# quadjr/aframe-gaussian-splatting

Measured on AMD Instinct MI355X. Metric: frames/sec @1920x1080 (sort+project+bin+blend per frame, 1M-splat train.splat-shaped scene), higher is better.
Workload: dtype f32

## Files before the change

### aframe-gaussian-splatting_amd/capi.py

```python
import ctypes as C
import os
import sys

import numpy as np

from . import build as _build

GS_OK = 0
E_BADARG, E_PLY_HEADER, E_PLY_PROP, E_HIP, E_OOM, E_NODEVICE, E_STATE, E_PLY_DATA, E_RETRY = -1, -2, -3, -4, -5, -6, -7, -8, -9
RENDER_FLIP_Y, RENDER_COUNT_FRAGS, RENDER_NO_EARLY_OUT, RENDER_ASYNC, RENDER_COUNT_EVALUATED = 1, 2, 4, 8, 16
OPT_PROFILE, OPT_TERMINATION, OPT_NEAR_PERMILLE, OPT_RECORD_STAGED, OPT_PIPELINE_DEPTH, OPT_WIDE_PAIRS, OPT_ENQUEUE_THREADS = 1, 2, 3, 4, 5, 6, 7
OPT_COMM_SELF_COPY = 8
OPT_BLEND_SPLIT = 9
OPT_FRAME_BATCH = 10
OPT_SORT_NEAR = 11
OPT_COMM_TRANSPORT = 12
OPT_AUTO_RETRY = 13
OPT_SORT_SHARE = 15
OPT_BINNING = 16
OPT_SUBTILE = 17
OPT_ROW_WALK = 18
OPT_SH_DEGREE = 19
OPT_ANTIALIAS = 20
OPT_SEG_COUNT = 21
OPT_SORT_NEAR_FORCE = 22
SORT_WHOLE, SORT_HISTOGRAM, SORT_SPEC, SORT_TAIL, SORT_STASH = 0, 1, 2, 3, 4
TRANSPORT_RCCL, TRANSPORT_INPROC = 0, 1
COMM_ID_BYTES = 128
BUF_CENTER_SCALE, BUF_COV_COLOR, BUF_SORT_ROWS, BUF_SORTED, BUF_PROJECTED, BUF_TILE_COUNT, BUF_TILE_STATS, BUF_UNSAT_MASK = 0, 1, 2, 3, 4, 5, 6, 7
BUF_SH = 8
BUF_STATE = 9
STATE_HIDDEN, STATE_SELECTED = 1, 2
SELECT_INVERT = 1

EXPORTS = [
    "gs_create", "gs_destroy", "gs_last_error", "gs_version", "gs_device_count", "gs_clear", "gs_push_splat", "gs_push_matrices", "gs_load_ply",
    "gs_ply_to_splat", "gs_ply_to_splat_gpu", "gs_count", "gs_sort", "gs_render", "gs_render_device", "gs_render_stereo", "gs_set_scene", "gs_sync",
    "gs_set_stream", "gs_frame_stream", "gs_frame_status_device", "gs_frame_lane", "gs_lane_stream", "gs_wait_stream", "gs_stream_wait_frame",
    "gs_model_view_matrix", "gs_projection_matrix", "gs_tick_uniforms", "gs_focal", "gs_scaled_size", "gs_set_option",
    "gs_get_stats", "gs_download",
    "gs_comm_unique_id", "gs_comm_init", "gs_comm_destroy", "gs_partition", "gs_render_gathered", "gs_read_gathered",
    "gs_host_alloc", "gs_host_free", "gs_sort_for", "gs_sort_gathered", "gs_gathered_size", "gs_sort_begin", "gs_sort_poll",
    "gs_create_multi", "gs_multi_destroy", "gs_multi_last_error", "gs_multi_devices", "gs_multi_ctx", "gs_multi_clear",
    "gs_multi_push_splat", "gs_multi_load_ply", "gs_multi_count", "gs_multi_set_option", "gs_multi_sort", "gs_multi_render",
    "gs_multi_render_device", "gs_multi_read", "gs_multi_sync",
    "gs_ply_sh", "gs_ply_sh_host", "gs_push_sh", "gs_sh_count", "gs_sh_eval", "gs_sh_eval_unrounded", "gs_camera_in_object", "gs_multi_push_sh",
    "gs_render_surface", "gs_render_surface_device", "gs_pick",
    "gs_antialias_factor",
    "gs_set_state", "gs_set_state_ids", "gs_state_count", "gs_select_box", "gs_select_sphere", "gs_select_rect", "gs_compact",
    "gs_sort_inspect",
    "gs_multi_set_state", "gs_multi_set_state_ids", "gs_multi_select_box", "gs_multi_select_sphere", "gs_multi_select_rect", "gs_multi_compact",
]
SURFACE_NONE = 0xFFFFFFFF

# ... 767 lines not shown
```

### aframe-gaussian-splatting_amd/csrc/gs_api.hip

```cpp
#include <stddef.h>
#include <stdlib.h>
#include <condition_variable>
#include <deque>
#include <functional>
#include <mutex>
#include <new>
#include <thread>
#include <set>
#include <vector>
#include "gs_internal.h"
#include "gs_ply.h"
#include "gs_sh.h"
#include "gs_host_tables.h"

static thread_local char g_create_err[512] = "";
thread_local char *gs_tl_err = nullptr;

#define CHECK_CTX(ctx) do { if (!(ctx)) return GS_E_BADARG; } while (0)
#define FAIL(code, ...) do { snprintf(GS_ERRBUF(ctx), GS_ERRLEN, __VA_ARGS__); return (code); } while (0)

template <typename T> static int dev_alloc(gs_ctx *ctx, T **p, size_t count)
{
    *p = nullptr;
    if (!count) count = 1;
// ... 711 lines not shown
}

GS_API const char *gs_last_error(const gs_ctx *ctx) { return ctx ? ctx->err : g_create_err; }

GS_API int gs_create(int device, gs_ctx **out)
{
    if (!out) return GS_E_BADARG;
    *out = nullptr;
    int ndev = 0;
    hipError_t e = hipGetDeviceCount(&ndev);
    if (e != hipSuccess || ndev <= 0) {
        snprintf(g_create_err, sizeof g_create_err, "no HIP device available (%s); this library has no CPU fallback",
                 e != hipSuccess ? hipGetErrorString(e) : "device count 0");
        return GS_E_NODEVICE;
    }
    if (device < 0 || device >= ndev) {
        snprintf(g_create_err, sizeof g_create_err, "device %d out of range (have %d)", device, ndev);
        return GS_E_BADARG;
    }
    gs_ctx *ctx = new (std::nothrow) gs_ctx();
    if (!ctx) { snprintf(g_create_err, sizeof g_create_err, "out of host memory"); return GS_E_OOM; }
    memset(ctx, 0, sizeof *ctx);
    ctx->device = device; ctx->renderable = true; ctx->t_eps = 1.0f / 1024.0f; gs_share_reset_create(ctx->share);
    ctx->lanes[0] = ctx; ctx->pipe_depth = 3; ctx->enqueue_threads = true; ctx->frame_batch = 1; ctx->exec = ctx; ctx->sort_near_opt = 1; ctx->auto_retry = true; ctx->subtile_opt = 1; ctx->row_walk_opt = 1; ctx->seg_count_opt = 1;
    { const char *e = getenv("GS_SPEC_STASH"); ctx->near_spec_opt = !(e && e[0] == '0'); }
#define CREATE_HIP(call) do { hipError_t _e = (call); if (_e != hipSuccess) {                                              \
        snprintf(g_create_err, sizeof g_create_err, "%s failed: %s", #call, hipGetErrorString(_e)); gs_destroy(ctx);      \
        return GS_E_HIP; } } while (0)
    CREATE_HIP(hipSetDevice(device));
    CREATE_HIP(init_frame_resources(ctx));
    {
        double tab[GS_POW10_ENTRIES];
        gs_build_pow10_table(tab);
        CREATE_HIP(hipMalloc((void **)&ctx->pow10tab, sizeof tab));
        CREATE_HIP(hipMemcpy(ctx->pow10tab, tab, sizeof tab, hipMemcpyHostToDevice));
    }
#undef CREATE_HIP
    *out = ctx;
    return GS_OK;
}

GS_API int gs_destroy(gs_ctx *ctx)
{
    if (!ctx) return GS_OK;
    (void)hipSetDevice(ctx->device);
    (void)gs_comm_destroy(ctx);
    for (int i = GS_MAX_LANES - 1; i >= 1; i--)
// ... 1157 lines not shown
        ctx->cur = 0; ctx->rot = 0; ctx->cur_async = false;
        return prepare_lanes(ctx);
    case GS_OPT_FRAME_BATCH:
        if (value != 1 && value != 2) FAIL(GS_E_BADARG, "frame batch must be 1 (off) or 2");
        GS_HIP(hipSetDevice(ctx->device));
        TRY(drain_all(ctx));
        ctx->frame_batch = (int)value;
        ctx->cur = 0; ctx->rot = 0; ctx->cur_async = false;
        return prepare_lanes(ctx);
    case GS_OPT_SUBTILE:
        if (value < 0 || value > 2) FAIL(GS_E_BADARG, "sub-tile lists: 0 (off), 1 (where splats are small) or 2 (always)");
        ctx->subtile_opt = (int)value;
        return GS_OK;
    case GS_OPT_ROW_WALK:
        if (value < 0 || value > 2) FAIL(GS_E_BADARG, "row walk: 0 (off), 1 (where splats are large) or 2 (always)");
        ctx->row_walk_opt = (int)value;
        return GS_OK;
    case GS_OPT_SEG_COUNT:
        if (value < 0 || value > 2) FAIL(GS_E_BADARG, "segment counts: 0 (never), 1 (where tile rows hold many runs) or 2 (always)");
        GS_HIP(hipSetDevice(ctx->device));
        TRY(drain_all(ctx));
        ctx->seg_count_opt = (int)value;
        return GS_OK;
    case GS_OPT_SH_DEGREE:
        if (value < 0 || value > GS_SH_MAX_DEGREE) FAIL(GS_E_BADARG, "spherical-harmonics degree: 0 (off) to 3");
        ctx->sh_opt = (int)value;
        return GS_OK;
    case GS_OPT_ANTIALIAS:
        if (value != 0 && value != 1) FAIL(GS_E_BADARG, "anti-aliased splats: 0 (off) or 1 (opacity compensated for the 0.3 px^2 dilation)");
        ctx->aa_opt = (int)value;
        return GS_OK;
    case GS_OPT_SORT_NEAR:
        if (value < 0 || value > 2) FAIL(GS_E_BADARG, "near-only sorts: 0 (off), 1 (scenes of 4 M splats and more) or 2 (always)");
        GS_HIP(hipSetDevice(ctx->device));
        TRY(drain_all(ctx));
        ctx->sort_near_opt = (int)value;
        return GS_OK;
    case GS_OPT_SORT_NEAR_FORCE:
        if (value < 0 || value > 0xFFFFFFFFll) FAIL(GS_E_BADARG, "forced near-only sorts: 0 (the policy decides) or the positions every sort without an index list is asked for");
        GS_HIP(hipSetDevice(ctx->device));
        TRY(drain_all(ctx));
        ctx->sort_near_force = (uint32_t)value;
        return GS_OK;
    default: FAIL(GS_E_BADARG, "unknown option %d", option);
    }
}
// ... 71 lines not shown
                                        hipMemcpyDeviceToHost));
        return GS_OK;
    }
    if (which == GS_BUF_STATE) {
        if (nbytes > ctx->edit_n) FAIL(GS_E_BADARG, "buffer %d holds %zu bytes, %zu requested", which, ctx->edit_n, nbytes);
        if (nbytes) GS_HIP(hipMemcpy(out, ctx->edit_state, nbytes, hipMemcpyDeviceToHost));
        return GS_OK;
    }
    if (which == GS_BUF_SH) {
        const size_t K = (size_t)gsm::sh_coefs(ctx->sh_deg), KS = (size_t)gsm::sh_channel_stride(ctx->sh_deg);
        if (nbytes > ctx->sh_n * 3 * K * 4 || nbytes % (K * 4)) FAIL(GS_E_BADARG, "buffer %d holds %zu bytes, %zu requested", which, ctx->sh_n * 3 * K * 4, nbytes);
        if (nbytes) GS_HIP(hipMemcpy2D(out, K * 4, ctx->sh, KS * 4, K * 4, nbytes / (K * 4), hipMemcpyDeviceToHost));
        return GS_OK;
    }
    switch (which) {
    case GS_BUF_SORT_ROWS: src = ctx->sort_rows; have = ctx->n * 16; break;
    case GS_BUF_SORTED:
        if (L->have_sort && L->sort_near_req) { TRY(lane_rc(ctx, L, ensure_full_sort(L))); GS_HIP(hipStreamSynchronize(L->stream)); }
        src = L->sorted; have = L->have_sort ? V * 4 : 0; break;
    case GS_BUF_PROJECTED: src = L->proj; have = L->have_sort ? V * 32 : 0; break;
    case GS_BUF_TILE_COUNT: src = L->tile_count; have = L->have_sort ? V * 4 : 0; break;
    case GS_BUF_TILE_STATS: src = L->tile_range; have = L->tile_cap * 8; break;
    case GS_BUF_UNSAT_MASK: src = L->unsat_mask; have = L->mask_cap * 4; break;
    default: FAIL(GS_E_BADARG, "unknown buffer %d", which);
    }
    if (nbytes > have) FAIL(GS_E_BADARG, "buffer %d holds %zu bytes, %zu requested", which, have, nbytes);
    if (nbytes && (!ctx->renderable && (which == GS_BUF_CENTER_SCALE || which == GS_BUF_COV_COLOR)))
        FAIL(GS_E_STATE, "context holds worker rows only");
    if (nbytes) GS_HIP(hipMemcpy(out, src, nbytes, hipMemcpyDeviceToHost));
    return GS_OK;
}

}
```

### aframe-gaussian-splatting_amd/csrc/gs_internal.h

```cpp
#pragma once
#include <hip/hip_runtime.h>
#include <stdint.h>
#include <stdio.h>
#include <string.h>
#include <type_traits>
#include "../../include/gs_splat.h"
#include "gs_device_math.h"
#include "gs_share.h"

#if defined(__HIP_DEVICE_COMPILE__) && !defined(__gfx950__)
#error "libgs_splat_hip is written for gfx950 (MI355X) only: build with --offload-arch=gfx950"
#endif

#define GS_TILE 16
#define GS_BLOCK 256
#define GS_CHUNK_S 2048
#define GS_CHUNK_L 4096
#ifndef GS_RADIX_LARGE_N
#define GS_RADIX_LARGE_N (3u << 20)
#endif
#define GS_RADIX_MAX_BINS 512
#define GS_TOUCH_PRIVATE_WORDS 16u
#define GS_STATUS_RING 64u
#define GS_NEED_WORDS 32u
// ... 157 lines not shown
    uint32_t *hist;  size_t hist_cap;
    uint32_t *radix_aux; size_t aux_cap;
    uint32_t *spine; size_t spine_cap;
    uint32_t *msd_grp; size_t msd_grp_cap;
    uint32_t *msd_tab;

    gsm::Projected *proj;
    uint2 *rect;
    uint32_t *tile_count;
    uint2 *emit_extra;
    float *zwin;
    float *scene_depth; uint32_t *scene_rgba; int scene_w, scene_h;
    uint2 *pair_a, *pair_b; size_t pair_cap;
    uint32_t blend_split_min;
    uint32_t pair_hint;
    uint32_t run_hint;
    uint32_t *row_cnt; size_t row_cnt_cap;
    uint2 *row_tot; size_t row_tot_cap;
    int *seg_diff;
    int bin_mode;
    int subtile_opt;
    int row_walk_opt;
    int seg_count_opt;
    uint32_t last_pairs, last_visible;
    uint2 *tile_range; size_t tile_cap;
    uint8_t *fb; size_t fb_cap;
    uint8_t *surf_buf; size_t surf_cap;
    struct GsComm *comm;
    uint8_t *gstage; size_t gstage_cap;
    uint8_t *gframe[2]; size_t gframe_cap[2];
    int gviews, gw[2], gh[2];
    float4 *state; size_t state_cap;
    uint32_t *unsat_mask; size_t mask_cap;
    GsShare share;
    GsShareLane share_lane;
    unsigned long long *part_min, *part_max;
    uint32_t *part_cnt, *part_valid, *part_vis;
    GsControl *ctl;
    GsControl *ctl_host;

    bool profile;
    bool profile_blend_only;
    uint32_t profile_every;
    uint32_t profile_tick;
    uint32_t record_staged;
    bool wide_pairs;
// ... 111 lines not shown
```

### aframe-gaussian-splatting_amd/csrc/gs_render.hip

```cpp
#include "gs_internal.h"
#include "gs_sh.h"

namespace {

#define GS_DPP_ADD(V, CTRL, ROWS) (V) += (uint32_t)__builtin_amdgcn_update_dpp(0, (int)(V), (CTRL), (ROWS), 0xF, false)
__device__ __forceinline__ uint32_t row16_sum(uint32_t v)
{
#ifdef GS_DEBUG_DPP_MAX
    const uint32_t v0_ = v;
#endif
    GS_DPP_ADD(v, 0xB1, 0xF);
    GS_DPP_ADD(v, 0x4E, 0xF);
    GS_DPP_ADD(v, 0x141, 0xF);
    GS_DPP_ADD(v, 0x140, 0xF);
#ifdef GS_DEBUG_DPP_MAX
    { uint32_t c = v0_; for (int m = 8; m >= 1; m >>= 1) c += __shfl_xor(c, m, 16); if (c != v) __builtin_trap(); }
#endif
    return v;
}
__device__ __forceinline__ uint32_t wave_sum(uint32_t v)
{
#ifdef GS_DEBUG_DPP_MAX
    uint32_t c_ = v; for (int m = 32; m >= 1; m >>= 1) c_ += __shfl_xor(c_, m, 64);
#endif
// ... 596 lines not shown
    __syncthreads();
    if (tid == 0) {
        const uint32_t total = I > 0xFFFFFFFFull ? 0xFFFFFFFFu : (uint32_t)I;
        ctl->vis_total = 0; ctl->n_emit_extra = 0;
        ctl->n_runs = (ROUND == 0 ? 0u : ctl->n_runs) + runs;
        if (ROUND == 0) { ctl->n_visible = 0; ctl->n_pairs_frame = 0; ctl->want_frame = 0; }
        else { ctl->unsat_round0 = ctl->unsat_count; if (ctl->unsat_count) ctl->unsat_events += 1; }
        ctl->j_lo = j_lo; ctl->j_hi = j_hi;
        ctl->scan_total = total;
        ctl->want_frame = (ctl->want_frame + total < total) ? 0xFFFFFFFFu : ctl->want_frame + total;
        if (ctl->want_frame > ctl->max_total) ctl->max_total = ctl->want_frame;
        if (total > pair_cap) { ctl->pair_overflow = 1; ctl->overflow_sticky = 1; ctl->n_pairs = 0; }
        else if (ROUND == 0) { ctl->pair_overflow = 0; ctl->n_pairs = total; }
        else ctl->n_pairs = ctl->pair_overflow ? 0u : total;
        ctl->n_visible += s_vis; ctl->n_pairs_frame += ctl->n_pairs;
        if (ROUND == 0 && near_count != 0xFFFFFFFFu) ctl->unsat_count = 0;
        if (last_round) {
            ctl->acc_frames += 1; ctl->acc_sorted += ctl->n_kept; ctl->acc_visible += ctl->n_visible; ctl->acc_pairs += ctl->n_pairs_frame;
        }
    }
    __syncthreads();
}

template <int ROUND>
__device__ __forceinline__ void k_emit_runs_body(const gsm::Projected *__restrict__ proj, const uint2 *__restrict__ rect,
                                                 const uint32_t *__restrict__ tile_count, const uint32_t *__restrict__ row_cnt,
                                                 const uint2 *__restrict__ row_tot, const GsFrameUniforms &u,
                                                 uint32_t *__restrict__ run_geom, uint32_t *__restrict__ run_ref,
                                                 const uint32_t *__restrict__ mask, GsControl *ctl, uint32_t pair_cap, uint2 *__restrict__ row_runs,
                                                 const uint32_t *__restrict__ part_vis, uint32_t nparts, int last_round)
{
    __shared__ float s_rec[GS_BLOCK][6];
    __shared__ uint32_t s_rows[GS_BLOCK], s_t[GS_BLOCK];
    __shared__ unsigned long long s_m[GS_BLOCK][4];
    __shared__ uint32_t s_rowrun[GS_BLOCK + 1], s_rowpair[GS_BLOCK + 1], s_base[GS_BLOCK];
    __shared__ uint32_t s_nbig, s_nmid;
    __shared__ unsigned long long s_p[4];
    const uint32_t tid = threadIdx.x;
    const int lane = threadIdx.x & 63, w = threadIdx.x >> 6;
    const uint32_t tiles_y = (uint32_t)u.tiles_y;
    const unsigned long long I = row_prefixes<false>(row_tot, tiles_y, s_rowrun, s_rowpair, nullptr, s_p);
    uint32_t j_lo, j_hi;
    round_range<ROUND>(ctl, u.near_count, j_lo, j_hi);
    const bool overflow = I > pair_cap || (ROUND == 1 && ctl->pair_overflow);
    if (blockIdx.x == 0) {
        round_books<ROUND>(ctl, I, s_rowrun[GS_BLOCK], j_lo, j_hi, u.near_count, part_vis, nparts, last_round, pair_cap);
        if (ROUND == 0 && tid < tiles_y) row_runs[tid] = make_uint2(s_rowrun[tid], overflow ? 0u : s_rowrun[tid + 1] - s_rowrun[tid]);
    }
    if (overflow) return;
    const uint32_t nchunks = (j_hi - j_lo + GS_BLOCK - 1) / GS_BLOCK;
    for (uint32_t c = blockIdx.x; c < nchunks; c += gridDim.x) {
        s_m[tid][0] = 0ull; s_m[tid][1] = 0ull; s_m[tid][2] = 0ull; s_m[tid][3] = 0ull;
        if (tid == 0) { s_nbig = 0; s_nmid = 0; }
        if (tid < tiles_y) s_base[tid] = s_rowrun[tid] + row_cnt[(size_t)tid * u.rc_stride + c];
        __syncthreads();
        const uint32_t j = j_lo + c * GS_BLOCK + tid;
        const uint32_t cnt = j < j_hi ? tile_count[j] : 0u;
        bool own = false;
        uint32_t ty0 = 0, ty1 = 0;
        gsm::Projected p;
        p.cx = p.cy = p.ax = p.ay = p.bx = p.by = 0.0f;
        uint32_t own_runs = 0, own_present = 0;
        if (cnt) {
            const uint2 rc = rect[j];
            if (rc.x & (1u << 14)) {
                own = true;
                ty0 = rc.x >> 16; ty1 = ty0 + ((rc.x >> 15) & 1u);
                own_runs = rc.y; own_present = (rc.x >> 12) & 3u;
            } else {
                const float4 *src = reinterpret_cast<const float4 *>(proj + j);
                const float4 ra = src[0]; const float2 rb = *reinterpret_cast<const float2 *>(src + 1);
                p.cx = ra.x; p.cy = ra.y; p.ax = ra.z; p.ay = ra.w; p.bx = rb.x; p.by = rb.y;
                ty0 = rc.x >> 16; ty1 = rc.y >> 16;
                const uint32_t q = (ty1 - ty0 >= 16) ? (GS_BLOCK - 1u - atomicAdd(&s_nbig, 1u)) : atomicAdd(&s_nmid, 1u);
                s_rec[q][0] = p.cx; s_rec[q][1] = p.cy; s_rec[q][2] = p.ax; s_rec[q][3] = p.ay; s_rec[q][4] = p.bx; s_rec[q][5] = p.by;
                s_rows[q] = ty0 | (ty1 << 16); s_t[q] = tid;
            }
        }
        __syncthreads();
        const uint32_t nmid = s_nmid, nbig = s_nbig;
#define GS_RUN_ONE(PP, EE, T, TY, FN) do { uint32_t a_, n_;                                                                       \
            gsm::splat_tile_row(PP, EE, (int)(TY), u.H, u.x0, u.x1b, a_, n_);                                                     \
            if (n_ && (ROUND == 0 || mask_count(mask + (TY) * u.mask_words, a_, n_))) { FN((T), (TY), a_, n_); } } while (0)
#define GS_RUN_PASS(FN) do {                                                                                                      \
            if (own) {                                                                                                            \
                for (uint32_t ty = ty0; ty <= ty1; ty++) if ((own_present >> (ty - ty0)) & 1u) {                                  \
                    const uint32_t r_ = own_runs >> (16u * (ty - ty0)), a_ = r_ & 0xFFu, n_ = ((r_ >> 8) & 0xFFu) + 1u;           \
                    if (ROUND == 0 || mask_count(mask + ty * u.mask_words, a_, n_)) { FN(tid, ty, a_, n_); } } }                  \
            for (uint32_t mi = (uint32_t)w * 4u + ((uint32_t)lane >> 4); mi < nmid; mi += 16u) {                                  \
                gsm::Projected q;                                                                                                 \
                q.cx = s_rec[mi][0]; q.cy = s_rec[mi][1]; q.ax = s_rec[mi][2]; q.ay = s_rec[mi][3]; q.bx = s_rec[mi][4]; q.by = s_rec[mi][5]; \
                gsm::EllipseRows e; gsm::ellipse_rows_setup(q, e);                                                                \
                const uint32_t ty = (s_rows[mi] & 0xFFFFu) + ((uint32_t)lane & 15u);                                              \
                if (ty <= (s_rows[mi] >> 16)) GS_RUN_ONE(q, e, s_t[mi], ty, FN); }                                                \
            for (uint32_t bq = (uint32_t)w; bq < nbig; bq += 4u) {                                                                \
                const uint32_t bi = GS_BLOCK - 1u - bq;                                                                           \
                gsm::Projected q;                                                                                                 \
                q.cx = s_rec[bi][0]; q.cy = s_rec[bi][1]; q.ax = s_rec[bi][2]; q.ay = s_rec[bi][3]; q.bx = s_rec[bi][4]; q.by = s_rec[bi][5]; \
                gsm::EllipseRows e; gsm::ellipse_rows_setup(q, e);                                                                \
                for (uint32_t ty = (s_rows[bi] & 0xFFFFu) + (uint32_t)lane; ty <= (s_rows[bi] >> 16); ty += 64u) GS_RUN_ONE(q, e, s_t[bi], ty, FN); } \
        } while (0)
#define GS_RUN_MARK(T, TY, A, N) atomicOr(&s_m[TY][(T) >> 6], 1ull << ((T) & 63u))
        GS_RUN_PASS(GS_RUN_MARK);
        __syncthreads();
#define GS_RUN_WRITE(T, TY, A, N) do { const uint32_t wq_ = (T) >> 6;                                                             \
            uint32_t rank_ = (uint32_t)__popcll(s_m[TY][wq_] & ((1ull << ((T) & 63u)) - 1ull));                                   \
            for (uint32_t k_ = 0; k_ < wq_; k_++) rank_ += (uint32_t)__popcll(s_m[TY][k_]);                                       \
            const uint32_t slot_ = s_base[TY] + rank_;                                                                            \
            run_geom[slot_] = (A) | ((N) << 16); run_ref[slot_] = j_lo + c * GS_BLOCK + (T); } while (0)
        GS_RUN_PASS(GS_RUN_WRITE);
#undef GS_RUN_WRITE
#undef GS_RUN_MARK
#undef GS_RUN_PASS
#undef GS_RUN_ONE
        __syncthreads();
    }
}

template <int ROUND>
__global__ __launch_bounds__(GS_BLOCK) void k_emit_runs(const gsm::Projected *__restrict__ proj, const uint2 *__restrict__ rect,
                                                        const uint32_t *__restrict__ tile_count, const uint32_t *__restrict__ row_cnt,
                                                        const uint2 *__restrict__ row_tot, GsFrameUniforms u,
                                                        uint32_t *__restrict__ run_geom, uint32_t *__restrict__ run_ref,
                                                        const uint32_t *__restrict__ mask, GsControl *ctl, uint32_t pair_cap, uint2 *__restrict__ row_runs,
                                                        const uint32_t *__restrict__ part_vis, uint32_t nparts, int last_round)
{
    k_emit_runs_body<ROUND>(proj, rect, tile_count, row_cnt, row_tot, u, run_geom, run_ref, mask, ctl, pair_cap, row_runs, part_vis, nparts, last_round);
}

template <int ROUND>
__device__ __forceinline__ void k_seg_count_body(const uint32_t *__restrict__ run_geom, const uint2 *__restrict__ row_tot, int *__restrict__ seg_diff,
                                                 const GsFrameUniforms &u, const GsControl *ctl, uint32_t pair_cap)
{
    __shared__ uint32_t s_rrun[GS_BLOCK + 1], s_rpair[GS_BLOCK + 1], s_item[GS_BLOCK + 1];
    __shared__ int s_d[GS_BLOCK + 1];
    __shared__ unsigned long long s_p[4];
    const uint32_t tid = threadIdx.x, tiles_y = (uint32_t)u.tiles_y;
    const unsigned long long I = row_prefixes<true>(row_tot, tiles_y, s_rrun, s_rpair, s_item, s_p);
    if (I > pair_cap || (ROUND == 1 && ctl->pair_overflow)) return;
    const uint32_t NI = s_item[GS_BLOCK];
    for (uint32_t item = blockIdx.x; item < NI; item += gridDim.x) {
        uint32_t row = 0;
#pragma unroll
        for (uint32_t step = GS_BLOCK / 2; step; step >>= 1) { const uint32_t t = row + step; if (t < tiles_y && s_item[t] <= item) row = t; }
        const uint32_t seg = item - s_item[row];
        const uint32_t rb = s_rrun[row], nr = s_rrun[row + 1] - rb;
        const uint32_t S = list_seg_len(nr), s0 = seg * S, s1 = min(nr, s0 + S);
        s_d[tid] = 0;
        if (tid == 0) s_d[GS_BLOCK] = 0;
        __syncthreads();
// ... 786 lines not shown
                (uint32_t)(fminf(fmaxf(o0, 0.0f), 1.0f) * 255.0f + 0.5f) | ((uint32_t)(fminf(fmaxf(o1, 0.0f), 1.0f) * 255.0f + 0.5f) << 8) |
                ((uint32_t)(fminf(fmaxf(o2, 0.0f), 1.0f) * 255.0f + 0.5f) << 16) | ((uint32_t)(fminf(fmaxf(o3, 0.0f), 1.0f) * 255.0f + 0.5f) << 24);
        }
        __syncthreads();
    }
#undef GS_PX_FETCH
#undef GS_WAVE_LDS_SYNC
}

template <int ROUND, bool SCENE>
__global__ __launch_bounds__(256) void k_blend_px(const uint2 *__restrict__ tile_range, const void *__restrict__ pairs,
                                                  const gsm::Projected *__restrict__ proj, GsFrameUniforms u,
                                                  uint8_t *__restrict__ out, float4 *__restrict__ state, uint32_t *__restrict__ mask,
                                                  const float *__restrict__ zwin, const float *__restrict__ scene_depth,
                                                  const uint32_t *__restrict__ scene_rgba, GsControl *ctl)
{
    k_blend_px_body<ROUND, SCENE>(tile_range, pairs, proj, u, out, state, mask, zwin, scene_depth, scene_rgba, ctl);
}

int bits_for(uint32_t n) { int b = 1; while (b < 32 && (1u << b) < n) b++; return b; }

template <int ROUND, bool RUNS, bool SH, bool AA> GS_BODY(F_project, (k_project<ROUND, RUNS, SH, AA>), (k_project_body<ROUND, RUNS, SH, AA>));
template <int ROUND> GS_BODY(F_row_scan, (k_row_scan<ROUND>), (k_row_scan_body<ROUND>));
template <int ROUND> GS_BODY(F_emit_runs, (k_emit_runs<ROUND>), (k_emit_runs_body<ROUND>));
template <int ROUND> GS_BODY(F_seg_count, (k_seg_count<ROUND>), (k_seg_count_body<ROUND>));
template <int ROUND, bool SEGC> GS_BODY(F_lists, (k_lists<ROUND, SEGC>), (k_lists_body<ROUND, SEGC>));
template <int ROUND> GS_BODY(F_pairs_check, (k_pairs_check<ROUND>), (k_pairs_check_body<ROUND>));
template <int ROUND> GS_BODY(F_emit, (k_emit<ROUND>), (k_emit_body<ROUND>));
GS_BODY(F_tile_ranges, (k_tile_ranges), (k_tile_ranges_body));
template <int ROUND, bool SCENE, bool SUB, bool WALK> GS_BODY(F_blend, (k_blend<false, ROUND, SCENE, SUB, WALK>), (k_blend_body<false, ROUND, SCENE, SUB, WALK>));
template <int ROUND, bool SCENE> GS_BODY(F_blend_px, (k_blend_px<ROUND, SCENE>), (k_blend_px_body<ROUND, SCENE>));
template <int ROUND, bool SCENE, bool SUB> GS_BODY(F_blend_count, (k_blend<true, ROUND, SCENE, SUB>), (k_blend_body<true, ROUND, SCENE, SUB>));
template <int ROUND, bool SCENE> GS_BODY(F_blend_surf, (k_blend_surf<ROUND, SCENE>), (k_blend_body<false, ROUND, SCENE, false, false, true>));


template <int ROUND, int NF>
int launch_blend(gs_ctx *const S[], const GsFrameUniforms V[], uint8_t *const out[], const void *const lists[])
{
    gs_ctx *ctx = S[0];
    const GsFrameUniforms &u = V[0];
    const uint32_t ntiles = (uint32_t)u.tiles_x * (uint32_t)u.tiles_y;
    hipStream_t st = ctx->stream;
    const uint32_t gb = ROUND == 1 ? (ntiles < 1024 ? ntiles : 1024) : ntiles;
    const bool scene = u.has_depth || u.has_scene_rgba;
    const bool count = (u.flags & GS_RENDER_COUNT_FRAGS) != 0;
    if (NF != 1 && (count || u.record_staged || u.surface)) { snprintf(GS_ERRBUF(ctx), GS_ERRLEN, "paired blend: a measurement or surface frame"); return GS_E_STATE; }
    GsFrameUniforms W[NF];
// ... 80 lines not shown
        gs_launch<NF, F_project<ROUND, RUNS, decltype(SH)::value, decltype(AA)::value>, GS_BLOCK>(g, st, 0, args);
    }); });
}

template <int ROUND, int NF>
int run_round_spans(gs_ctx *const S[], const GsFrameUniforms U[], uint8_t *const out[], bool last_round, uint32_t g, uint32_t stride)
{
    gs_ctx *ctx = S[0];
    const GsFrameUniforms &u = U[0];
    hipStream_t st = ctx->stream;
    for (int k = 0; k < NF; k++) { const int rcc = gs_ensure_row_tables(S[k], (size_t)stride * (size_t)u.tiles_y); if (rcc != GS_OK) return rcc; }
    GsFrameUniforms V[NF];
    uint32_t *geom[NF], *ref[NF], *lists[NF];
    for (int k = 0; k < NF; k++) {
        V[k] = U[k];
        V[k].rc_stride = stride;
        V[k].row_walk = row_walk_round<ROUND>(u) ? 1u : 0u;
        V[k].walk_ref = (uint32_t)S[k]->pair_cap;
        geom[k] = reinterpret_cast<uint32_t *>(S[k]->pair_a); ref[k] = geom[k] + S[k]->pair_cap; lists[k] = reinterpret_cast<uint32_t *>(S[k]->pair_b);
    }
    launch_project<ROUND, true, NF>(S, V, g);
    GS_HIP(hipGetLastError());
    if (ROUND == 0) GS_PROF_RECORD(ctx, 3);
    gs_launch<NF, F_row_scan<ROUND>, GS_BLOCK>((uint32_t)u.tiles_y, st, 0, [&](int k) {
        return gs_pack_make(S[k]->row_cnt, S[k]->row_tot, (const GsControl *)S[k]->ctl, U[k].near_count, stride, (uint32_t)u.tiles_y, S[k]->unsat_mask, u.mask_words); });
    gs_launch<NF, F_emit_runs<ROUND>, GS_BLOCK>(g, st, 0, [&](int k) {
        return gs_pack_make((const gsm::Projected *)S[k]->proj, (const uint2 *)S[k]->rect, (const uint32_t *)S[k]->tile_count, (const uint32_t *)S[k]->row_cnt,
                            (const uint2 *)S[k]->row_tot, V[k], geom[k], ref[k], (const uint32_t *)S[k]->unsat_mask, S[k]->ctl, (uint32_t)S[k]->pair_cap,
                            S[k]->row_tot + GS_BLOCK, (const uint32_t *)S[k]->part_vis, g, last_round ? 1 : 0); });
    const void *fpairs[NF];
    if (V[0].row_walk) {
        GS_HIP(hipGetLastError());
        if (ROUND == 0) GS_PROF_RECORD(ctx, 4);
        for (int k = 0; k < NF; k++) fpairs[k] = geom[k];
        return launch_blend<ROUND, NF>(S, V, out, fpairs);
    }
    uint32_t gl = (uint32_t)u.tiles_y * GS_LIST_SEGS; if (gl > (ROUND == 1 ? 512u : 2048u)) gl = ROUND == 1 ? 512u : 2048u;
    const int segc_opt = gs_root(ctx)->seg_count_opt;
    const bool segc = ROUND == 0 && segc_opt != 0 &&
                      (segc_opt == 2 || __atomic_load_n(&gs_root(ctx)->run_hint, __ATOMIC_RELAXED) > GS_SEGC_RUNS_PER_ROW * (uint32_t)u.tiles_y);
    if (segc) for (int k = 0; k < NF; k++) S[k]->stats.seg_count = 1u;
    if (segc)
        gs_launch<NF, F_seg_count<ROUND>, GS_BLOCK>(gl, st, 0, [&](int k) {
            return gs_pack_make((const uint32_t *)geom[k], (const uint2 *)S[k]->row_tot, S[k]->seg_diff, V[k], (const GsControl *)S[k]->ctl, (uint32_t)S[k]->pair_cap); });
    gs_flag(segc, [&](auto SEGC) {
        gs_launch<NF, F_lists<ROUND, decltype(SEGC)::value>, GS_BLOCK>(gl, st, 0, [&](int k) {
            return gs_pack_make((const uint32_t *)geom[k], (const uint32_t *)ref[k], (const uint2 *)S[k]->row_tot, (const int *)S[k]->seg_diff, lists[k], S[k]->tile_range, V[k],
                                (const uint32_t *)S[k]->unsat_mask, (const GsControl *)S[k]->ctl, (uint32_t)S[k]->pair_cap); }); });
    GS_HIP(hipGetLastError());
    if (ROUND == 0) GS_PROF_RECORD(ctx, 4);
    for (int k = 0; k < NF; k++) fpairs[k] = lists[k];
    return launch_blend<ROUND, NF>(S, V, out, fpairs);
// ... 136 lines not shown
```

### include/gs_splat.h

```cpp
#ifndef GS_SPLAT_H
#define GS_SPLAT_H

#include <stddef.h>
#include <stdint.h>

#ifdef __cplusplus
extern "C" {
#endif

#define GS_API __attribute__((visibility("default")))

typedef struct gs_ctx gs_ctx;

typedef enum gs_status {
    GS_OK = 0,
    GS_E_BADARG = -1,
    GS_E_PLY_HEADER = -2,
    GS_E_PLY_PROP = -3,
    GS_E_HIP = -4,
    GS_E_OOM = -5,
    GS_E_NODEVICE = -6,
    GS_E_STATE = -7,
    GS_E_PLY_DATA = -8,
    GS_E_RETRY = -9
// ... 183 lines not shown
    uint32_t binning;
    uint32_t sh_degree;
    uint32_t n_hidden;
    uint32_t surface;
    uint32_t antialias;
    uint32_t seg_count;
    uint32_t n_runs;
} gs_stats;

#define GS_OPT_PROFILE 1
#define GS_OPT_TERMINATION 2
#define GS_OPT_NEAR_PERMILLE 3
#define GS_OPT_RECORD_STAGED 4
#define GS_OPT_PIPELINE_DEPTH 5
#define GS_OPT_WIDE_PAIRS 6
#define GS_OPT_BINNING 16
#define GS_OPT_SUBTILE 17
#define GS_OPT_ROW_WALK 18
#define GS_OPT_SH_DEGREE 19
#define GS_OPT_ANTIALIAS 20
#define GS_OPT_SEG_COUNT 21
#define GS_OPT_ENQUEUE_THREADS 7
#define GS_OPT_SORT_NEAR_FORCE 22
GS_API int gs_set_option(gs_ctx *ctx, int option, int64_t value);
GS_API int gs_get_stats(gs_ctx *ctx, gs_stats *out);

typedef struct gs_sort_info {
    uint32_t form;
    uint32_t near_req;
    uint32_t n_kept;
    uint32_t n_valid;
    uint32_t n_records;
    uint32_t order_incomplete;
    uint32_t near_overflow;
    uint32_t spec_fail;
    uint32_t threshold_bin;
    uint32_t reserved[3];
} gs_sort_info;
GS_API int gs_sort_inspect(gs_ctx *ctx, gs_sort_info *info, uint32_t *out_idx, size_t cap);

#define GS_BUF_CENTER_SCALE 0
#define GS_BUF_COV_COLOR 1
#define GS_BUF_SORT_ROWS 2
#define GS_BUF_SORTED 3
#define GS_BUF_PROJECTED 4
#define GS_BUF_TILE_COUNT 5
#define GS_BUF_TILE_STATS 6
#define GS_BUF_UNSAT_MASK 7
#define GS_BUF_SH 8
#define GS_BUF_STATE 9
GS_API int gs_download(gs_ctx *ctx, int which, void *out, size_t nbytes);

#ifdef __cplusplus
}
#endif
#endif
```

Before: 20810.

## Fold row-count prefix sums into k_emit_runs and keep first run results in registers

Adds a default-on option that skips the separate k_row_scan launch when the chunk count is small. Each k_emit_runs block now sums the per-row chunk counts itself, clears the unsaturated mask and writes row_tot. The mark/write passes are also rewritten so the first few mid and big splat runs per thread stay in registers instead of being recomputed in the write pass. This removes one kernel launch and some ellipse re-evaluation per frame, at the cost of every block redundantly reading the row_cnt table and holding more registers.

Measured after the change: 20460. 0.983x the previous value.

```diff
diff --git a/aframe-gaussian-splatting_amd/capi.py b/aframe-gaussian-splatting_amd/capi.py
--- a/aframe-gaussian-splatting_amd/capi.py
+++ b/aframe-gaussian-splatting_amd/capi.py
@@ -24,12 +24,14 @@
 OPT_ANTIALIAS = 20
 OPT_SEG_COUNT = 21
 OPT_SORT_NEAR_FORCE = 22
+OPT_BIN_FOLD = 23
 SORT_WHOLE, SORT_HISTOGRAM, SORT_SPEC, SORT_TAIL, SORT_STASH = 0, 1, 2, 3, 4
 TRANSPORT_RCCL, TRANSPORT_INPROC = 0, 1
 COMM_ID_BYTES = 128
 BUF_CENTER_SCALE, BUF_COV_COLOR, BUF_SORT_ROWS, BUF_SORTED, BUF_PROJECTED, BUF_TILE_COUNT, BUF_TILE_STATS, BUF_UNSAT_MASK = 0, 1, 2, 3, 4, 5, 6, 7
 BUF_SH = 8
 BUF_STATE = 9
+BUF_RUN_GEOM, BUF_RUN_REF, BUF_ROW_TOT = 10, 11, 12
 STATE_HIDDEN, STATE_SELECTED = 1, 2
 SELECT_INVERT = 1
 
diff --git a/aframe-gaussian-splatting_amd/csrc/gs_api.hip b/aframe-gaussian-splatting_amd/csrc/gs_api.hip
--- a/aframe-gaussian-splatting_amd/csrc/gs_api.hip
+++ b/aframe-gaussian-splatting_amd/csrc/gs_api.hip
@@ -757,7 +757,7 @@
     if (!ctx) { snprintf(g_create_err, sizeof g_create_err, "out of host memory"); return GS_E_OOM; }
     memset(ctx, 0, sizeof *ctx);
     ctx->device = device; ctx->renderable = true; ctx->t_eps = 1.0f / 1024.0f; gs_share_reset_create(ctx->share);
-    ctx->lanes[0] = ctx; ctx->pipe_depth = 3; ctx->enqueue_threads = true; ctx->frame_batch = 1; ctx->exec = ctx; ctx->sort_near_opt = 1; ctx->auto_retry = true; ctx->subtile_opt = 1; ctx->row_walk_opt = 1; ctx->seg_count_opt = 1;
+    ctx->lanes[0] = ctx; ctx->pipe_depth = 3; ctx->enqueue_threads = true; ctx->frame_batch = 1; ctx->exec = ctx; ctx->sort_near_opt = 1; ctx->auto_retry = true; ctx->subtile_opt = 1; ctx->row_walk_opt = 1; ctx->seg_count_opt = 1; ctx->bin_fold_opt = 1;
     { const char *e = getenv("GS_SPEC_STASH"); ctx->near_spec_opt = !(e && e[0] == '0'); }
 #define CREATE_HIP(call) do { hipError_t _e = (call); if (_e != hipSuccess) {                                              \
         snprintf(g_create_err, sizeof g_create_err, "%s failed: %s", #call, hipGetErrorString(_e)); gs_destroy(ctx);      \
@@ -1961,6 +1961,12 @@
         TRY(drain_all(ctx));
         ctx->seg_count_opt = (int)value;
         return GS_OK;
+    case GS_OPT_BIN_FOLD:
+        if (value != 0 && value != 1) FAIL(GS_E_BADARG, "folded run emit: 0 (k_row_scan, then k_emit_runs) or 1 (small rounds: k_emit_runs sums the row counts itself)");
+        GS_HIP(hipSetDevice(ctx->device));
+        TRY(drain_all(ctx));
+        ctx->bin_fold_opt = (int)value;
+        return GS_OK;
     case GS_OPT_SH_DEGREE:
         if (value < 0 || value > GS_SH_MAX_DEGREE) FAIL(GS_E_BADARG, "spherical-harmonics degree: 0 (off) to 3");
         ctx->sh_opt = (int)value;
@@ -2078,6 +2084,9 @@
     case GS_BUF_TILE_COUNT: src = L->tile_count; have = L->have_sort ? V * 4 : 0; break;
     case GS_BUF_TILE_STATS: src = L->tile_range; have = L->tile_cap * 8; break;
     case GS_BUF_UNSAT_MASK: src = L->unsat_mask; have = L->mask_cap * 4; break;
+    case GS_BUF_RUN_GEOM: src = L->pair_a; have = L->pair_a ? L->pair_cap * 4 : 0; break;
+    case GS_BUF_RUN_REF: src = L->pair_a ? (const uint32_t *)L->pair_a + L->pair_cap : nullptr; have = L->pair_a ? L->pair_cap * 4 : 0; break;
+    case GS_BUF_ROW_TOT: src = L->row_tot; have = L->row_tot ? L->row_tot_cap * 8 : 0; break;
     default: FAIL(GS_E_BADARG, "unknown buffer %d", which);
     }
     if (nbytes > have) FAIL(GS_E_BADARG, "buffer %d holds %zu bytes, %zu requested", which, have, nbytes);
diff --git a/aframe-gaussian-splatting_amd/csrc/gs_internal.h b/aframe-gaussian-splatting_amd/csrc/gs_internal.h
--- a/aframe-gaussian-splatting_amd/csrc/gs_internal.h
+++ b/aframe-gaussian-splatting_amd/csrc/gs_internal.h
@@ -203,6 +203,7 @@
     int subtile_opt;
     int row_walk_opt;
     int seg_count_opt;
+    int bin_fold_opt;
     uint32_t last_pairs, last_visible;
     uint2 *tile_range; size_t tile_cap;
     uint8_t *fb; size_t fb_cap;
diff --git a/aframe-gaussian-splatting_amd/csrc/gs_render.hip b/aframe-gaussian-splatting_amd/csrc/gs_render.hip
--- a/aframe-gaussian-splatting_amd/csrc/gs_render.hip
+++ b/aframe-gaussian-splatting_amd/csrc/gs_render.hip
@@ -642,37 +642,76 @@
     __syncthreads();
 }
 
-template <int ROUND>
+#define GS_FOLD_MAX_POS 65536u
+static_assert(GS_FOLD_MAX_POS / GS_BLOCK <= 16u * 16u && (unsigned long long)(GS_FOLD_MAX_POS / GS_BLOCK) << 23 <= 0xFFFFFFFFull, "the folded row sums");
+__device__ __forceinline__ void fold_row_sums(const uint32_t *__restrict__ row_cnt, uint32_t rc_stride, uint32_t tiles_y, uint32_t nch, uint32_t c,
+                                              uint2 *s_tot, uint32_t *s_pre)
+{
+    const uint32_t l16 = threadIdx.x & 15u, grp = threadIdx.x >> 4;
+    for (uint32_t rb = 0; rb < tiles_y; rb += 32u) {
+        uint32_t v[2][16];
+#pragma unroll
+        for (uint32_t b = 0; b < 2; b++)
+#pragma unroll
+            for (uint32_t k = 0; k < 16; k++) {
+                const uint32_t row = rb + 16u * b + grp, ch = l16 + 16u * k;
+                v[b][k] = (row < tiles_y && ch < nch) ? row_cnt[(size_t)row * rc_stride + ch] : 0u;
+            }
+#pragma unroll
+        for (uint32_t b = 0; b < 2; b++) {
+            uint32_t sr = 0, sp = 0, pre = 0;
+#pragma unroll
+            for (uint32_t k = 0; k < 16; k++) { const uint32_t r = v[b][k] & 0x1FFu; sr += r; sp += v[b][k] >> 9; pre += l16 + 16u * k < c ? r : 0u; }
+            sr = row16_sum(sr); sp = row16_sum(sp); pre = row16_sum(pre);
+            const uint32_t row = rb + 16u * b + grp;
+            if (l16 == 0 && row < tiles_y) { s_tot[row] = make_uint2(sr, sp); s_pre[row] = pre; }
+        }
+    }
+    __syncthreads();
+}
+
+#define GS_RUN_KEEP 4u
+template <int ROUND, bool FOLD>
 __device__ __forceinline__ void k_emit_runs_body(const gsm::Projected *__restrict__ proj, const uint2 *__restrict__ rect,
                                                  const uint32_t *__restrict__ tile_count, const uint32_t *__restrict__ row_cnt,
-                                                 const uint2 *__restrict__ row_tot, const GsFrameUniforms &u,
+                                                 uint2 *__restrict__ row_tot, const GsFrameUniforms &u,
                                                  uint32_t *__restrict__ run_geom, uint32_t *__restrict__ run_ref,
-                                                 const uint32_t *__restrict__ mask, GsControl *ctl, uint32_t pair_cap, uint2 *__restrict__ row_runs,
+                                                 uint32_t *__restrict__ mask, GsControl *ctl, uint32_t pair_cap, uint2 *__restrict__ row_runs,
                                                  const uint32_t *__restrict__ part_vis, uint32_t nparts, int last_round)
 {
     __shared__ float s_rec[GS_BLOCK][6];
     __shared__ uint32_t s_rows[GS_BLOCK], s_t[GS_BLOCK];
     __shared__ unsigned long long s_m[GS_BLOCK][4];
     __shared__ uint32_t s_rowrun[GS_BLOCK + 1], s_rowpair[GS_BLOCK + 1], s_base[GS_BLOCK];
+    __shared__ uint2 s_tot[FOLD ? GS_BLOCK : 1];
+    __shared__ uint32_t s_pre[FOLD ? GS_BLOCK : 1];
     __shared__ uint32_t s_nbig, s_nmid;
     __shared__ unsigned long long s_p[4];
     const uint32_t tid = threadIdx.x;
     const int lane = threadIdx.x & 63, w = threadIdx.x >> 6;
     const uint32_t tiles_y = (uint32_t)u.tiles_y;
-    const unsigned long long I = row_prefixes<false>(row_tot, tiles_y, s_rowrun, s_rowpair, nullptr, s_p);
     uint32_t j_lo, j_hi;
     round_range<ROUND>(ctl, u.near_count, j_lo, j_hi);
+    const uint32_t nchunks = (j_hi - j_lo + GS_BLOCK - 1) / GS_BLOCK;
+    if (FOLD) {
+        if (ROUND == 0) for (uint32_t row = blockIdx.x; row < tiles_y; row += gridDim.x)
+            for (uint32_t i = tid; i < u.mask_words; i += GS_BLOCK) mask[row * u.mask_words + i] = 0u;
+        fold_row_sums(row_cnt, u.rc_stride, tiles_y, nchunks, blockIdx.x, s_tot, s_pre);
+    }
+    const unsigned long long I = row_prefixes<false>(FOLD ? (const uint2 *)s_tot : (const uint2 *)row_tot, tiles_y, s_rowrun, s_rowpair, nullptr, s_p);
     const bool overflow = I > pair_cap || (ROUND == 1 && ctl->pair_overflow);
     if (blockIdx.x == 0) {
         round_books<ROUND>(ctl, I, s_rowrun[GS_BLOCK], j_lo, j_hi, u.near_count, part_vis, nparts, last_round, pair_cap);
         if (ROUND == 0 && tid < tiles_y) row_runs[tid] = make_uint2(s_rowrun[tid], overflow ? 0u : s_rowrun[tid + 1] - s_rowrun[tid]);
+        if (FOLD && tid < tiles_y) row_tot[tid] = s_tot[tid];
     }
     if (overflow) return;
-    const uint32_t nchunks = (j_hi - j_lo + GS_BLOCK - 1) / GS_BLOCK;
+    const uint32_t l16 = (uint32_t)lane & 15u, mbase = (uint32_t)w * 4u + ((uint32_t)lane >> 4);
     for (uint32_t c = blockIdx.x; c < nchunks; c += gridDim.x) {
+        if (FOLD && c != blockIdx.x) fold_row_sums(row_cnt, u.rc_stride, tiles_y, nchunks, c, s_tot, s_pre);
         s_m[tid][0] = 0ull; s_m[tid][1] = 0ull; s_m[tid][2] = 0ull; s_m[tid][3] = 0ull;
         if (tid == 0) { s_nbig = 0; s_nmid = 0; }
-        if (tid < tiles_y) s_base[tid] = s_rowrun[tid] + row_cnt[(size_t)tid * u.rc_stride + c];
+        if (tid < tiles_y) s_base[tid] = s_rowrun[tid] + (FOLD ? s_pre[tid] : row_cnt[(size_t)tid * u.rc_stride + c]);
         __syncthreads();
         const uint32_t j = j_lo + c * GS_BLOCK + tid;
         const uint32_t cnt = j < j_hi ? tile_count[j] : 0u;
@@ -699,53 +738,102 @@
         }
         __syncthreads();
         const uint32_t nmid = s_nmid, nbig = s_nbig;
-#define GS_RUN_ONE(PP, EE, T, TY, FN) do { uint32_t a_, n_;                                                                       \
-            gsm::splat_tile_row(PP, EE, (int)(TY), u.H, u.x0, u.x1b, a_, n_);                                                     \
-            if (n_ && (ROUND == 0 || mask_count(mask + (TY) * u.mask_words, a_, n_))) { FN((T), (TY), a_, n_); } } while (0)
-#define GS_RUN_PASS(FN) do {                                                                                                      \
-            if (own) {                                                                                                            \
-                for (uint32_t ty = ty0; ty <= ty1; ty++) if ((own_present >> (ty - ty0)) & 1u) {                                  \
-                    const uint32_t r_ = own_runs >> (16u * (ty - ty0)), a_ = r_ & 0xFFu, n_ = ((r_ >> 8) & 0xFFu) + 1u;           \
-                    if (ROUND == 0 || mask_count(mask + ty * u.mask_words, a_, n_)) { FN(tid, ty, a_, n_); } } }                  \
-            for (uint32_t mi = (uint32_t)w * 4u + ((uint32_t)lane >> 4); mi < nmid; mi += 16u) {                                  \
-                gsm::Projected q;                                                                                                 \
-                q.cx = s_rec[mi][0]; q.cy = s_rec[mi][1]; q.ax = s_rec[mi][2]; q.ay = s_rec[mi][3]; q.bx = s_rec[mi][4]; q.by = s_rec[mi][5]; \
-                gsm::EllipseRows e; gsm::ellipse_rows_setup(q, e);                                                                \
-                const uint32_t ty = (s_rows[mi] & 0xFFFFu) + ((uint32_t)lane & 15u);                                              \
-                if (ty <= (s_rows[mi] >> 16)) GS_RUN_ONE(q, e, s_t[mi], ty, FN); }                                                \
-            for (uint32_t bq = (uint32_t)w; bq < nbig; bq += 4u) {                                                                \
-                const uint32_t bi = GS_BLOCK - 1u - bq;                                                                           \
-                gsm::Projected q;                                                                                                 \
-                q.cx = s_rec[bi][0]; q.cy = s_rec[bi][1]; q.ax = s_rec[bi][2]; q.ay = s_rec[bi][3]; q.bx = s_rec[bi][4]; q.by = s_rec[bi][5]; \
-                gsm::EllipseRows e; gsm::ellipse_rows_setup(q, e);                                                                \
-                for (uint32_t ty = (s_rows[bi] & 0xFFFFu) + (uint32_t)lane; ty <= (s_rows[bi] >> 16); ty += 64u) GS_RUN_ONE(q, e, s_t[bi], ty, FN); } \
-        } while (0)
-#define GS_RUN_MARK(T, TY, A, N) atomicOr(&s_m[TY][(T) >> 6], 1ull << ((T) & 63u))
-        GS_RUN_PASS(GS_RUN_MARK);
-        __syncthreads();
-#define GS_RUN_WRITE(T, TY, A, N) do { const uint32_t wq_ = (T) >> 6;                                                             \
-            uint32_t rank_ = (uint32_t)__popcll(s_m[TY][wq_] & ((1ull << ((T) & 63u)) - 1ull));                                   \
-            for (uint32_t k_ = 0; k_ < wq_; k_++) rank_ += (uint32_t)__popcll(s_m[TY][k_]);                                       \
-            const uint32_t slot_ = s_base[TY] + rank_;                                                                            \
-            run_geom[slot_] = (A) | ((N) << 16); run_ref[slot_] = j_lo + c * GS_BLOCK + (T); } while (0)
-        GS_RUN_PASS(GS_RUN_WRITE);
-#undef GS_RUN_WRITE
-#undef GS_RUN_MARK
-#undef GS_RUN_PASS
-#undef GS_RUN_ONE
-        __syncthreads();
-    }
-}
-
-template <int ROUND>
+        const auto run_of = [&](uint32_t qi, uint32_t ty) -> uint32_t {
+            gsm::Projected q;
+            q.cx = s_rec[qi][0]; q.cy = s_rec[qi][1]; q.ax = s_rec[qi][2]; q.ay = s_rec[qi][3]; q.bx = s_rec[qi][4]; q.by = s_rec[qi][5];
+            gsm::EllipseRows e; gsm::ellipse_rows_setup(q, e);
+            uint32_t a_, n_;
+            gsm::splat_tile_row(q, e, (int)ty, u.H, u.x0, u.x1b, a_, n_);
+            return (n_ && (ROUND == 0 || mask_count(mask + ty * u.mask_words, a_, n_))) ? (a_ | (n_ << 16)) : 0u;
+        };
+        const auto mark = [&](uint32_t t, uint32_t ty) { atomicOr(&s_m[ty][t >> 6], 1ull << (t & 63u)); };
+        const auto write = [&](uint32_t t, uint32_t ty, uint32_t g) {
+            const uint32_t wq = t >> 6;
+            uint32_t rank = (uint32_t)__popcll(s_m[ty][wq] & ((1ull << (t & 63u)) - 1ull));
+            for (uint32_t k = 0; k < wq; k++) rank += (uint32_t)__popcll(s_m[ty][k]);
+            const uint32_t slot = s_base[ty] + rank;
+            run_geom[slot] = g; run_ref[slot] = j_lo + c * GS_BLOCK + t;
+        };
+        if (ROUND == 1 && own) {
+            for (uint32_t ty = ty0; ty <= ty1; ty++) if ((own_present >> (ty - ty0)) & 1u) {
+                const uint32_t r_ = own_runs >> (16u * (ty - ty0)), a_ = r_ & 0xFFu, n_ = ((r_ >> 8) & 0xFFu) + 1u;
+                if (!mask_count(mask + ty * u.mask_words, a_, n_)) own_present &= ~(1u << (ty - ty0));
+            }
+        }
+        if (own) for (uint32_t ty = ty0; ty <= ty1; ty++) if ((own_present >> (ty - ty0)) & 1u) mark(tid, ty);
+        uint32_t kmid[GS_RUN_KEEP], kbig[GS_RUN_KEEP];
+#pragma unroll
+        for (uint32_t i = 0; i < GS_RUN_KEEP; i++) {
+            const uint32_t mi = mbase + 16u * i;
+            kmid[i] = 0u;
+            if (mi < nmid) {
+                const uint32_t ty = (s_rows[mi] & 0xFFFFu) + l16;
+                if (ty <= (s_rows[mi] >> 16)) kmid[i] = run_of(mi, ty);
+                if (kmid[i]) mark(s_t[mi], ty);
+            }
+        }
+        for (uint32_t mi = mbase + 16u * GS_RUN_KEEP; mi < nmid; mi += 16u) {
+            const uint32_t ty = (s_rows[mi] & 0xFFFFu) + l16;
+            if (ty <= (s_rows[mi] >> 16) && run_of(mi, ty)) mark(s_t[mi], ty);
+        }
+#pragma unroll
+        for (uint32_t i = 0; i < GS_RUN_KEEP; i++) {
+            const uint32_t bq = (uint32_t)w + 4u * i;
+            kbig[i] = 0u;
+            if (bq < nbig) {
+                const uint32_t bi = GS_BLOCK - 1u - bq, last = s_rows[bi] >> 16;
+                uint32_t ty = (s_rows[bi] & 0xFFFFu) + (uint32_t)lane;
+                if (ty <= last) kbig[i] = run_of(bi, ty);
+                if (kbig[i]) mark(s_t[bi], ty);
+                for (ty += 64u; ty <= last; ty += 64u) if (run_of(bi, ty)) mark(s_t[bi], ty);
+            }
+        }
+        for (uint32_t bq = (uint32_t)w + 4u * GS_RUN_KEEP; bq < nbig; bq += 4u) {
+            const uint32_t bi = GS_BLOCK - 1u - bq;
+            for (uint32_t ty = (s_rows[bi] & 0xFFFFu) + (uint32_t)lane; ty <= (s_rows[bi] >> 16); ty += 64u) if (run_of(bi, ty)) mark(s_t[bi], ty);
+        }
+        __syncthreads();
+        if (own) for (uint32_t ty = ty0; ty <= ty1; ty++) if ((own_present >> (ty - ty0)) & 1u) {
+            const uint32_t r_ = own_runs >> (16u * (ty - ty0));
+            write(tid, ty, (r_ & 0xFFu) | ((((r_ >> 8) & 0xFFu) + 1u) << 16));
+        }
+#pragma unroll
+        for (uint32_t i = 0; i < GS_RUN_KEEP; i++) {
+            const uint32_t mi = mbase + 16u * i;
+            if (kmid[i]) write(s_t[mi], (s_rows[mi] & 0xFFFFu) + l16, kmid[i]);
+        }
+        for (uint32_t mi = mbase + 16u * GS_RUN_KEEP; mi < nmid; mi += 16u) {
+            const uint32_t ty = (s_rows[mi] & 0xFFFFu) + l16;
+            const uint32_t g = ty <= (s_rows[mi] >> 16) ? run_of(mi, ty) : 0u;
+            if (g) write(s_t[mi], ty, g);
+        }
+#pragma unroll
+        for (uint32_t i = 0; i < GS_RUN_KEEP; i++) {
+            const uint32_t bq = (uint32_t)w + 4u * i;
+            if (bq < nbig) {
+                const uint32_t bi = GS_BLOCK - 1u - bq, last = s_rows[bi] >> 16;
+                uint32_t ty = (s_rows[bi] & 0xFFFFu) + (uint32_t)lane;
+                if (kbig[i]) write(s_t[bi], ty, kbig[i]);
+                for (ty += 64u; ty <= last; ty += 64u) { const uint32_t g = run_of(bi, ty); if (g) write(s_t[bi], ty, g); }
+            }
+        }
+        for (uint32_t bq = (uint32_t)w + 4u * GS_RUN_KEEP; bq < nbig; bq += 4u) {
+            const uint32_t bi = GS_BLOCK - 1u - bq;
+            for (uint32_t ty = (s_rows[bi] & 0xFFFFu) + (uint32_t)lane; ty <= (s_rows[bi] >> 16); ty += 64u) { const uint32_t g = run_of(bi, ty); if (g) write(s_t[bi], ty, g); }
+        }
+        __syncthreads();
+    }
+}
+
+template <int ROUND, bool FOLD>
 __global__ __launch_bounds__(GS_BLOCK) void k_emit_runs(const gsm::Projected *__restrict__ proj, const uint2 *__restrict__ rect,
                                                         const uint32_t *__restrict__ tile_count, const uint32_t *__restrict__ row_cnt,
-                                                        const uint2 *__restrict__ row_tot, GsFrameUniforms u,
+                                                        uint2 *__restrict__ row_tot, GsFrameUniforms u,
                                                         uint32_t *__restrict__ run_geom, uint32_t *__restrict__ run_ref,
-                                                        const uint32_t *__restrict__ mask, GsControl *ctl, uint32_t pair_cap, uint2 *__restrict__ row_runs,
+                                                        uint32_t *__restrict__ mask, GsControl *ctl, uint32_t pair_cap, uint2 *__restrict__ row_runs,
                                                         const uint32_t *__restrict__ part_vis, uint32_t nparts, int last_round)
 {
-    k_emit_runs_body<ROUND>(proj, rect, tile_count, row_cnt, row_tot, u, run_geom, run_ref, mask, ctl, pair_cap, row_runs, part_vis, nparts, last_round);
+    k_emit_runs_body<ROUND, FOLD>(proj, rect, tile_count, row_cnt, row_tot, u, run_geom, run_ref, mask, ctl, pair_cap, row_runs, part_vis, nparts, last_round);
 }
 
 template <int ROUND>
@@ -1578,7 +1666,7 @@
 
 template <int ROUND, bool RUNS, bool SH, bool AA> GS_BODY(F_project, (k_project<ROUND, RUNS, SH, AA>), (k_project_body<ROUND, RUNS, SH, AA>));
 template <int ROUND> GS_BODY(F_row_scan, (k_row_scan<ROUND>), (k_row_scan_body<ROUND>));
-template <int ROUND> GS_BODY(F_emit_runs, (k_emit_runs<ROUND>), (k_emit_runs_body<ROUND>));
+template <int ROUND, bool FOLD> GS_BODY(F_emit_runs, (k_emit_runs<ROUND, FOLD>), (k_emit_runs_body<ROUND, FOLD>));
 template <int ROUND> GS_BODY(F_seg_count, (k_seg_count<ROUND>), (k_seg_count_body<ROUND>));
 template <int ROUND, bool SEGC> GS_BODY(F_lists, (k_lists<ROUND, SEGC>), (k_lists_body<ROUND, SEGC>));
 template <int ROUND> GS_BODY(F_pairs_check, (k_pairs_check<ROUND>), (k_pairs_check_body<ROUND>));
@@ -1705,12 +1793,15 @@
     launch_project<ROUND, true, NF>(S, V, g);
     GS_HIP(hipGetLastError());
     if (ROUND == 0) GS_PROF_RECORD(ctx, 3);
-    gs_launch<NF, F_row_scan<ROUND>, GS_BLOCK>((uint32_t)u.tiles_y, st, 0, [&](int k) {
-        return gs_pack_make(S[k]->row_cnt, S[k]->row_tot, (const GsControl *)S[k]->ctl, U[k].near_count, stride, (uint32_t)u.tiles_y, S[k]->unsat_mask, u.mask_words); });
-    gs_launch<NF, F_emit_runs<ROUND>, GS_BLOCK>(g, st, 0, [&](int k) {
-        return gs_pack_make((const gsm::Projected *)S[k]->proj, (const uint2 *)S[k]->rect, (const uint32_t *)S[k]->tile_count, (const uint32_t *)S[k]->row_cnt,
-                            (const uint2 *)S[k]->row_tot, V[k], geom[k], ref[k], (const uint32_t *)S[k]->unsat_mask, S[k]->ctl, (uint32_t)S[k]->pair_cap,
-                            S[k]->row_tot + GS_BLOCK, (const uint32_t *)S[k]->part_vis, g, last_round ? 1 : 0); });
+    const bool fold = gs_root(ctx)->bin_fold_opt != 0 && (size_t)(stride - 1u) * GS_BLOCK <= GS_FOLD_MAX_POS && g >= stride - 1u;
+    if (!fold)
+        gs_launch<NF, F_row_scan<ROUND>, GS_BLOCK>((uint32_t)u.tiles_y, st, 0, [&](int k) {
+            return gs_pack_make(S[k]->row_cnt, S[k]->row_tot, (const GsControl *)S[k]->ctl, U[k].near_count, stride, (uint32_t)u.tiles_y, S[k]->unsat_mask, u.mask_words); });
+    gs_flag(fold, [&](auto FOLD) {
+        gs_launch<NF, F_emit_runs<ROUND, decltype(FOLD)::value>, GS_BLOCK>(g, st, 0, [&](int k) {
+            return gs_pack_make((const gsm::Projected *)S[k]->proj, (const uint2 *)S[k]->rect, (const uint32_t *)S[k]->tile_count, (const uint32_t *)S[k]->row_cnt,
+                                S[k]->row_tot, V[k], geom[k], ref[k], S[k]->unsat_mask, S[k]->ctl, (uint32_t)S[k]->pair_cap,
+                                S[k]->row_tot + GS_BLOCK, (const uint32_t *)S[k]->part_vis, g, last_round ? 1 : 0); }); });
     const void *fpairs[NF];
     if (V[0].row_walk) {
         GS_HIP(hipGetLastError());
diff --git a/include/gs_splat.h b/include/gs_splat.h
--- a/include/gs_splat.h
+++ b/include/gs_splat.h
@@ -229,6 +229,7 @@
 #define GS_OPT_SEG_COUNT 21
 #define GS_OPT_ENQUEUE_THREADS 7
 #define GS_OPT_SORT_NEAR_FORCE 22
+#define GS_OPT_BIN_FOLD 23
 GS_API int gs_set_option(gs_ctx *ctx, int option, int64_t value);
 GS_API int gs_get_stats(gs_ctx *ctx, gs_stats *out);
 
@@ -256,6 +257,9 @@
 #define GS_BUF_UNSAT_MASK 7
 #define GS_BUF_SH 8
 #define GS_BUF_STATE 9
+#define GS_BUF_RUN_GEOM 10
+#define GS_BUF_RUN_REF 11
+#define GS_BUF_ROW_TOT 12
 GS_API int gs_download(gs_ctx *ctx, int which, void *out, size_t nbytes);
 
 #ifdef __cplusplus
```
